# Kimahriman/hdfs-native

Hardware: AMD Instinct MI355X
Metric: GiB/s device-resident RS(6,3) encode+decode, 1 MiB cells, at 1/2/4/8 MI355X (higher is better)
Workload: dtype u8

## Files before the change

hdfs-native_amd/csrc/ec_kernels.hip:

```cpp
#include <hip/hip_runtime.h>

#include <dlfcn.h>

#include <algorithm>
#include <cstdint>
#include <functional>
#include <map>
#include <memory>
#include <mutex>
#include <thread>
#include <tuple>
#include <vector>

#include "bitslice.hpp"
#include "ec_kernels.hpp"
#include "gf_device.hpp"
#include "work_queue.hpp"
#include "xor_networks.hpp"

namespace hec {

template <int K, int R, int U, bool NT, int BS, int WQ = 0>
__global__ __launch_bounds__(BS) void gf_matmul_v16(MatmulArgs a) {
    static_assert(WQ == 0 || K > 0, "the work queue needs compile-time k");
    __shared__ PermTable s_tab[R][kMaxK];
    __shared__ uint8_t s_exp[512];
    __shared__ uint8_t s_log[256];
    __shared__ uint8_t s_coef[R * kMaxK];
    const int k = K ? K : a.k;
    prologue<R, BS>(a, k, s_tab, s_exp, s_log, s_coef);

    const uint32_t chunks = a.chunks;
    const uint32_t total = a.total_tiles;
    constexpr uint32_t TILE = WQ ? 64 * U : BS * U;
    constexpr uint32_t USTEP = WQ ? 64 : BS;
    const uint32_t lcol = WQ ? (threadIdx.x & 63u) : threadIdx.x;

    u32x4 acc[U][R];
#pragma unroll
    for (int u = 0; u < U; u++)
#pragma unroll
        for (int j = 0; j < R; j++) acc[u][j] = u32x4{0, 0, 0, 0};
    const uint32_t wq_n = gridDim.x < kMixedQueues ? gridDim.x : kMixedQueues;
    const uint32_t wq_q = blockIdx.x % wq_n;
    uint32_t* const wq_ctr = WQ ? a.queue + wq_q * (kMixedQueueStride / 4) : nullptr;
    if constexpr (WQ > 0) queue_zero_next(a.queue_zero);
    uint32_t wq_next, wq_round = 0, wq_left = 0;
    asm volatile("" : "=v"(wq_next));
    auto next_tile = [&]() -> uint32_t {
        for (;;) {
            if (wq_left == 0) {
                const uint32_t v = uint32_t(__builtin_amdgcn_readfirstlane(int(wq_next)));
                wq_round = v * uint32_t(WQ);
                wq_left = WQ;
                if (uint64_t(wq_round) * wq_n + wq_q >= total) return total;
                if ((threadIdx.x & 63u) == 0) wq_next = atomicAdd(wq_ctr, 1u);
            } else {
                wq_round++;
            }
            wq_left--;
            const uint64_t t = uint64_t(wq_round) * wq_n + wq_q;
            if (t < total) return uint32_t(t);
            wq_left = 0;
        }
    };
    if constexpr (WQ > 0)
        if ((threadIdx.x & 63u) == 0) wq_next = atomicAdd(wq_ctr, 1u);
    for (uint32_t tile = WQ ? next_tile() : blockIdx.x; tile < total; tile = WQ ? next_tile() : tile + gridDim.x) {
        uint32_t stripe, tcol;
        tile_coords(tile, a, stripe, tcol);
        asm volatile("" ::: "memory");
        if constexpr (K > 0) {
            u32x4 x[U][K];
            bool live[U];
            uint32_t offs[U];
#pragma unroll
            for (int u = 0; u < U; u++) {
                const uint32_t col = tcol * TILE + u * USTEP + lcol;
                live[u] = col < chunks;
                offs[u] = (live[u] ? col : 0u) * 16u;
            }
#pragma unroll
            for (int u = 0; u < U; u++)
#pragma unroll
                for (int i = 0; i < K; i++)
                    x[u][i] = load16<NT>((a.in[i] + uint64_t(stripe) * a.in_stride[i]) + offs[u]);
#pragma unroll
            for (int u = 0; u < U; u++)
#pragma unroll
                for (int j = 0; j < R; j++) asm volatile("" ::"v"(acc[u][j]));
            __builtin_amdgcn_sched_barrier(0);
#pragma unroll
            for (int i = 0; i < K; i++) {
                uint32_t toff = uint32_t(i) * uint32_t(sizeof(PermTable));
                asm volatile("" : "+v"(toff));
                if (i > 0) {
#pragma unroll
                    for (int u = 0; u < U; u++)
#pragma unroll
                        for (int j = 0; j < R; j++) asm volatile("" : "+v"(acc[u][j]) : "v"(toff));
                }
                Sel s[U][4];
#pragma unroll
                for (int u = 0; u < U; u++)
#pragma unroll
                    for (int d = 0; d < 4; d++) s[u][d] = make_sel(x[u][i][d]);
#pragma unroll
                for (int j = 0; j < R; j++) {
                    const PermTable& t =
                        *reinterpret_cast<const PermTable*>(reinterpret_cast<const char*>(&s_tab[j][0]) + toff);
                    const uint32_t t0lo = t.t0lo, t0hi = t.t0hi, t1lo = t.t1lo, t1hi = t.t1hi, t2 = t.t2;
#pragma unroll
                    for (int u = 0; u < U; u++)
#pragma unroll
                        for (int d = 0; d < 4; d++) {
                            const uint32_t p = gf_mul4(t0lo, t0hi, t1lo, t1hi, t2, s[u][d].s0, s[u][d].s1, s[u][d].s2);
                            acc[u][j][d] = i == 0 ? p : (acc[u][j][d] ^ p);
                        }
                }
                __builtin_amdgcn_sched_barrier(0);
            }
#pragma unroll
            for (int u = 0; u < U; u++)
#pragma unroll
                for (int j = 0; j < R; j++) asm volatile("" : "+v"(acc[u][j]));
            if ((tcol + 1) * TILE <= chunks) {
#pragma unroll
                for (int u = 0; u < U; u++)
#pragma unroll
                    for (int j = 0; j < R; j++)
                        store16<NT>((a.out[j] + uint64_t(stripe) * a.out_stride[j]) + offs[u], acc[u][j]);
            } else {
#pragma unroll
                for (int u = 0; u < U; u++) {
                    if (!live[u]) continue;
#pragma unroll
                    for (int j = 0; j < R; j++)
                        store16<NT>((a.out[j] + uint64_t(stripe) * a.out_stride[j]) + offs[u], acc[u][j]);
                }
            }
            if (a.drain) asm volatile("s_waitcnt vmcnt(0)" ::: "memory");
        } else {
#pragma unroll
            for (int u = 0; u < U; u++) {
                const uint32_t col = tcol * TILE + u * BS + threadIdx.x;
                if (col >= chunks) continue;
                const uint64_t off = uint64_t(col) * 16u;
                u32x4 racc[R];
#pragma unroll
                for (int j = 0; j < R; j++) racc[j] = u32x4{0, 0, 0, 0};
                for (int i = 0; i < k; i++) {
                    u32x4 x = load16<NT>(a.in[i] + uint64_t(stripe) * a.in_stride[i] + off);
                    Sel s[4];
#pragma unroll
                    for (int d = 0; d < 4; d++) s[d] = make_sel(x[d]);
#pragma unroll
                    for (int j = 0; j < R; j++) {
                        const PermTable& t = s_tab[j][i];
                        const uint32_t t0lo = t.t0lo, t0hi = t.t0hi, t1lo = t.t1lo, t1hi = t.t1hi, t2 = t.t2;
#pragma unroll
                        for (int d = 0; d < 4; d++)
                            racc[j][d] ^= gf_mul4(t0lo, t0hi, t1lo, t1hi, t2, s[d].s0, s[d].s1, s[d].s2);
                    }
                }
#pragma unroll
                for (int j = 0; j < R; j++) store16<NT>(a.out[j] + uint64_t(stripe) * a.out_stride[j] + off, racc[j]);
            }
        }
    }
}

template <int K, int R, int U, int BS>
__global__ __launch_bounds__(BS) void gf_encode_bsl(MatmulArgs a) {
    static_assert(bitslice::rs_net_available<K, R>() && U % 2 == 0, "bit-sliced RS encode");
    constexpr int G = U / 2;
    const uint32_t chunks = a.chunks;
    const uint32_t total = a.total_tiles;
    constexpr uint32_t TILE = BS * U;
    u32x4 acc[U][R];
#pragma unroll
    for (int u = 0; u < U; u++)
#pragma unroll
        for (int j = 0; j < R; j++) acc[u][j] = u32x4{0, 0, 0, 0};
    for (uint32_t tile = blockIdx.x; tile < total; tile += gridDim.x) {
        uint32_t stripe, tcol;
        tile_coords(tile, a, stripe, tcol);
        u32x4 x[U][K];
        bool live[U];
        uint32_t offs[U];
#pragma unroll
        for (int u = 0; u < U; u++) {
            const uint32_t col = tcol * TILE + u * BS + threadIdx.x;
            live[u] = col < chunks;
            offs[u] = (live[u] ? col : 0u) * 16u;
        }
#pragma unroll
        for (int u = 0; u < U; u++)
#pragma unroll
            for (int i = 0; i < K; i++) x[u][i] = load16<true>((a.in[i] + uint64_t(stripe) * a.in_stride[i]) + offs[u]);
#pragma unroll
        for (int u = 0; u < U; u++)
#pragma unroll
            for (int j = 0; j < R; j++) asm volatile("" ::"v"(acc[u][j]));
        __builtin_amdgcn_sched_barrier(0);
        uint32_t accp[G][R * 8];
#pragma unroll
        for (int i = 0; i < K; i++) {
#pragma unroll
            for (int g = 0; g < G; g++) {
                uint32_t pl[8] = {x[2 * g][i][0],     x[2 * g][i][1],     x[2 * g][i][2],     x[2 * g][i][3],
                                  x[2 * g + 1][i][0], x[2 * g + 1][i][1], x[2 * g + 1][i][2], x[2 * g + 1][i][3]};
                if (i > 0) {
#pragma unroll
                    for (int t = 0; t < R * 8; t++) asm volatile("" : "+v"(accp[g][t]));
                }
                bitslice::transpose8(pl);
                bitslice::rs_absorb_at<K, R>(i, pl, accp[g]);
                __builtin_amdgcn_sched_barrier(0);
            }
        }
#pragma unroll
        for (int g = 0; g < G; g++)
#pragma unroll
            for (int j = 0; j < R; j++) {
                uint32_t q[8];
#pragma unroll
                for (int t = 0; t < 8; t++) q[t] = accp[g][8 * j + t];
                bitslice::transpose8(q);
                acc[2 * g][j] = u32x4{q[0], q[1], q[2], q[3]};
                acc[2 * g + 1][j] = u32x4{q[4], q[5], q[6], q[7]};
            }
#pragma unroll
        for (int u = 0; u < U; u++)
#pragma unroll
            for (int j = 0; j < R; j++) asm volatile("" : "+v"(acc[u][j]));
        if ((tcol + 1) * TILE <= chunks) {
#pragma unroll
            for (int u = 0; u < U; u++)
#pragma unroll
                for (int j = 0; j < R; j++)
                    store16<true>((a.out[j] + uint64_t(stripe) * a.out_stride[j]) + offs[u], acc[u][j]);
        } else {
#pragma unroll
            for (int u = 0; u < U; u++) {
                if (!live[u]) continue;
#pragma unroll
                for (int j = 0; j < R; j++)
                    store16<true>((a.out[j] + uint64_t(stripe) * a.out_stride[j]) + offs[u], acc[u][j]);
            }
        }
        if (a.drain) asm volatile("s_waitcnt vmcnt(0)" ::: "memory");
    }
}

template <int K, int R, int U, int BS, bool BSL = false>
__global__ __launch_bounds__(BS) void gf_matmul_dma(MatmulArgs a) {
    static_assert(K > 0, "DMA kernel needs a compile-time input count");
    static_assert(!BSL || (bitslice::rs_net_available<K, R>() && U % 2 == 0), "bit-sliced RS encode");
    constexpr int WAVES = BS / 64;
    constexpr int PIECE = 1024;
    constexpr int STAGE = WAVES * K * U * PIECE;
    constexpr int TAB = R * kMaxK * int(sizeof(PermTable));
    __shared__ __attribute__((aligned(16))) uint8_t s_mem[STAGE + TAB + 512 + 256 + R * kMaxK];
    PermTable(*s_tab)[kMaxK] = reinterpret_cast<PermTable(*)[kMaxK]>(s_mem + STAGE);
    uint8_t* s_exp = s_mem + STAGE + TAB;
    uint8_t* s_log = s_exp + 512;
    uint8_t* s_coef = s_log + 256;
    prologue<R, BS>(a, K, s_tab, s_exp, s_log, s_coef);

    const uint32_t chunks = a.chunks;
    const uint32_t total = a.total_tiles;
    constexpr uint32_t TILE = BS * U;
    const int wave = __builtin_amdgcn_readfirstlane(threadIdx.x / 64);
    const int lane = threadIdx.x & 63;
    uint8_t* stage = s_mem + wave * (K * U * PIECE);

    auto issue = [&](uint32_t tile) {
        uint32_t stripe, tcol;
        tile_coords(tile, a, stripe, tcol);
#pragma unroll
        for (int u = 0; u < U; u++) {
            uint32_t col = tcol * TILE + u * BS + wave * 64 + lane;
            col = col < chunks ? col : chunks - 1;
            const uint32_t off = col * 16u;
#pragma unroll
            for (int i = 0; i < K; i++) {
                const uint8_t* src = (a.in[i] + uint64_t(stripe) * a.in_stride[i]) + off;
                __builtin_amdgcn_global_load_lds(
                    reinterpret_cast<const void*>(src),
                    (__attribute__((address_space(3))) void*)(stage + (i * U + u) * PIECE), 16, 0,
                    2 );
            }
        }
    };

    uint32_t tile = blockIdx.x;
    if (tile < total) issue(tile);
    bool prev_full = false;
    for (; tile < total; tile += gridDim.x) {
        if (prev_full)
            asm volatile("s_waitcnt vmcnt(%0)" ::"n"(R * U) : "memory");
        else
            asm volatile("s_waitcnt vmcnt(0)" ::: "memory");
        u32x4 x[U][K];
#pragma unroll
        for (int u = 0; u < U; u++)
#pragma unroll
            for (int i = 0; i < K; i++)
                x[u][i] = *reinterpret_cast<const u32x4*>(stage + (i * U + u) * PIECE + lane * 16);
        asm volatile("s_waitcnt lgkmcnt(0)" ::: "memory");
        __builtin_amdgcn_sched_barrier(0);
        const uint32_t next = tile + gridDim.x;
        if (next < total) issue(next);
        __builtin_amdgcn_sched_barrier(0);

        uint32_t stripe, tcol;
        tile_coords(tile, a, stripe, tcol);
        u32x4 acc[U][R];
        if constexpr (BSL) {
            constexpr int G = U / 2;
            uint32_t accp[G][R * 8];
#pragma unroll
            for (int i = 0; i < K; i++) {
#pragma unroll
                for (int g = 0; g < G; g++) {
                    uint32_t pl[8] = {x[2 * g][i][0],     x[2 * g][i][1],     x[2 * g][i][2],     x[2 * g][i][3],
                                      x[2 * g + 1][i][0], x[2 * g + 1][i][1], x[2 * g + 1][i][2], x[2 * g + 1][i][3]};
                    if (i > 0) {
#pragma unroll
                        for (int t = 0; t < R * 8; t++) asm volatile("" : "+v"(accp[g][t]));
                    }
                    bitslice::transpose8(pl);
                    bitslice::rs_absorb_at<K, R>(i, pl, accp[g]);
                    __builtin_amdgcn_sched_barrier(0);
                }
            }
#pragma unroll
            for (int g = 0; g < G; g++)
#pragma unroll
                for (int j = 0; j < R; j++) {
                    uint32_t q[8];
#pragma unroll
                    for (int t = 0; t < 8; t++) q[t] = accp[g][8 * j + t];
                    bitslice::transpose8(q);
                    acc[2 * g][j] = u32x4{q[0], q[1], q[2], q[3]};
                    acc[2 * g + 1][j] = u32x4{q[4], q[5], q[6], q[7]};
                }
        } else {
#pragma unroll
        for (int u = 0; u < U; u++)
#pragma unroll
            for (int j = 0; j < R; j++) acc[u][j] = u32x4{0, 0, 0, 0};
#pragma unroll
        for (int i = 0; i < K; i++) {
            uint32_t toff = uint32_t(i) * uint32_t(sizeof(PermTable));
            asm volatile("" : "+v"(toff));
#pragma unroll
            for (int u = 0; u < U; u++)
#pragma unroll
                for (int j = 0; j < R; j++) asm volatile("" : "+v"(acc[u][j]) : "v"(toff));
            Sel sl[U][4];
#pragma unroll
            for (int u = 0; u < U; u++)
#pragma unroll
                for (int d = 0; d < 4; d++) sl[u][d] = make_sel(x[u][i][d]);
#pragma unroll
            for (int j = 0; j < R; j++) {
                const PermTable& t =
                    *reinterpret_cast<const PermTable*>(reinterpret_cast<const char*>(&s_tab[j][0]) + toff);
                const uint32_t t0lo = t.t0lo, t0hi = t.t0hi, t1lo = t.t1lo, t1hi = t.t1hi, t2 = t.t2;
#pragma unroll
                for (int u = 0; u < U; u++)
#pragma unroll
                    for (int d = 0; d < 4; d++)
                        acc[u][j][d] ^= gf_mul4(t0lo, t0hi, t1lo, t1hi, t2, sl[u][d].s0, sl[u][d].s1, sl[u][d].s2);
            }
            __builtin_amdgcn_sched_barrier(0);
        }
        }
        const bool full = __builtin_amdgcn_readfirstlane(
                              int(tcol * TILE + (U - 1) * BS + wave * 64 + 63 < chunks)) != 0;
        if (full) {
#pragma unroll
            for (int u = 0; u < U; u++) {
                const uint32_t off = (tcol * TILE + u * BS + threadIdx.x) * 16u;
#pragma unroll
                for (int j = 0; j < R; j++)
                    store16<true>((a.out[j] + uint64_t(stripe) * a.out_stride[j]) + off, acc[u][j]);
            }
        } else {
#pragma unroll
            for (int u = 0; u < U; u++) {
                const uint32_t col = tcol * TILE + u * BS + threadIdx.x;
                if (col >= chunks) continue;
                const uint32_t off = col * 16u;
#pragma unroll
                for (int j = 0; j < R; j++)
                    store16<true>((a.out[j] + uint64_t(stripe) * a.out_stride[j]) + off, acc[u][j]);
            }
        }
        prev_full = full;
    }
    asm volatile("s_waitcnt vmcnt(0)" ::: "memory");
}

template <int K, int R, int U, int BS, bool RESIDENT, bool MIXED_SKIP = true, int WQ = 0>
__global__ __launch_bounds__(BS) void gf_decode_mixed(MixedArgs a) {
    static_assert(WQ == 0 || RESIDENT, "the work queue needs resident plans");
    static_assert(K > 0, "compile-time k");
    __shared__ PermTable s_tab[RESIDENT ? 1 : R][K];
    __shared__ DevPlanHeader s_hdr;
    __shared__ uint64_t s_base[kMaxShards], s_stride[kMaxShards], s_obase[kMaxK], s_ostride[kMaxK];
    extern __shared__ __attribute__((aligned(16))) uint8_t s_dyn[];
    const int tid = threadIdx.x;
    if (tid < kMaxShards) {
        s_base[tid] = reinterpret_cast<uint64_t>(a.base[tid]);
        s_stride[tid] = a.stride[tid];
    }
    if (tid < kMaxK) {
        s_obase[tid] = reinterpret_cast<uint64_t>(a.out[tid]);
        s_ostride[tid] = a.out_stride[tid];
    }
    const uint32_t off_bytes = (uint32_t(a.stripes) * 4u + 15u) & ~15u;
    if constexpr (RESIDENT) {
        const uint32_t off_words = uint32_t(a.stripes);
        for (uint32_t t = tid; t < off_words; t += BS) reinterpret_cast<uint32_t*>(s_dyn)[t] = a.stripe_off[t];
        const uint32_t words = a.blob_bytes / 4;
        for (uint32_t t = tid; t < words; t += BS)
            reinterpret_cast<uint32_t*>(s_dyn + off_bytes)[t] = reinterpret_cast<const uint32_t*>(a.plans)[t];
    }
    __syncthreads();
    const uint32_t chunks = a.chunks;
    const uint32_t total = a.total_tiles;
    constexpr uint32_t TILE = WQ ? 64 * U : BS * U;
    constexpr uint32_t USTEP = WQ ? 64 : BS;
    const uint32_t lcol = WQ ? (threadIdx.x & 63u) : threadIdx.x;
    MatmulArgs order;
    order.tiles_per_stripe = a.tiles_per_stripe;
    order.group = a.group;
    order.grouped_tiles = a.grouped_tiles;
    order.stripes = a.stripes;

    uint32_t t_begin = blockIdx.x, t_end = total, t_step = gridDim.x;
    if constexpr (!RESIDENT) {
        const uint32_t per = (total + gridDim.x - 1) / gridDim.x;
        t_begin = blockIdx.x * per;
        t_end = min(total, t_begin + per);
        t_step = 1;
        order.group = 1;
    }
    uint32_t cur_stripe = 0xFFFFFFFFu;
    bool cur_none = true;
    u32x4 acc[U][R];
#pragma unroll
    for (int u = 0; u < U; u++)
#pragma unroll
        for (int j = 0; j < R; j++) acc[u][j] = u32x4{0, 0, 0, 0};
    auto run_tile = [&](uint32_t tile) {
        uint32_t stripe, tcol;
        tile_coords(tile, order, stripe, tcol);
        const DevPlanHeader* hdr = &s_hdr;
        const PermTable* tabs = &s_tab[0][0];
        if constexpr (RESIDENT) {
            const uint32_t off = __builtin_amdgcn_readfirstlane(reinterpret_cast<const uint32_t*>(s_dyn)[stripe]);
            if (off == kNoPlan) return;
            hdr = reinterpret_cast<const DevPlanHeader*>(s_dyn + off_bytes + off);
            tabs = reinterpret_cast<const PermTable*>(s_dyn + off_bytes + off + sizeof(DevPlanHeader)) + a.row0 * K;
        } else {
            if (stripe != cur_stripe) {
                __syncthreads();
// ... 547 lines not shown
Shape default_shape(int k, uint64_t cell_len) {
    if (k > 6) return {2, 512, 8, true, false};
    (void)k;
    (void)cell_len;
    return {4, 256, 1, true, false};
}

}

namespace {

constexpr size_t kSetBytes = size_t(kMixedQueues) * kMixedQueueStride;
constexpr size_t kMaxStreamSets = 4096;
constexpr size_t kGraphSets = 256;

struct StreamSets {
    std::mutex mu;
    uint32_t* set[2] = {nullptr, nullptr};
    unsigned cur = 0;
    bool zeroed = false;
};

struct DeviceQueues {
    std::mutex mu;
    std::map<unsigned long long, std::unique_ptr<StreamSets>> streams;
    std::vector<std::unique_ptr<StreamSets>> thread_sets;
    uint32_t* graph_pool = nullptr;
    size_t graph_next = 0;
    bool reserved = false;
};

DeviceQueues& device_queues(int device) {
    static std::mutex mu;
    static std::map<int, std::unique_ptr<DeviceQueues>> all;
    std::lock_guard<std::mutex> lk(mu);
    auto& d = all[device];
    if (!d) d.reset(new DeviceQueues);
    return *d;
}

}

QueueLease::QueueLease(QueueLease&& o) noexcept : use(o.use), zero(o.zero), st_(o.st_) {
    o.use = o.zero = nullptr;
    o.st_ = nullptr;
}

QueueLease& QueueLease::operator=(QueueLease&& o) noexcept {
    if (this != &o) {
        if (st_) static_cast<StreamSets*>(st_)->mu.unlock();
        use = o.use;
        zero = o.zero;
        st_ = o.st_;
        o.use = o.zero = nullptr;
        o.st_ = nullptr;
    }
    return *this;
}

QueueLease::~QueueLease() {
    if (st_) static_cast<StreamSets*>(st_)->mu.unlock();
}

void QueueLease::launched() {
    if (st_) static_cast<StreamSets*>(st_)->cur ^= 1u;
}

void queue_reserve(int device) {
    DeviceQueues& d = device_queues(device);
    std::lock_guard<std::mutex> lk(d.mu);
    if (d.reserved) return;
    d.reserved = true;
    void* p = nullptr;
    if (hipMalloc(&p, kGraphSets * kSetBytes) != hipSuccess) {
        (void)hipGetLastError();
        return;
    }
    d.graph_pool = static_cast<uint32_t*>(p);
}

void queue_stats(int device, uint64_t* streams, uint64_t* graph_sets) {
    DeviceQueues& d = device_queues(device);
    std::lock_guard<std::mutex> lk(d.mu);
    if (streams) *streams = d.streams.size() + d.thread_sets.size();
    if (graph_sets) *graph_sets = d.graph_next;
}

namespace {

typedef hipError_t (*StreamGetIdFn)(hipStream_t, unsigned long long*);

StreamGetIdFn stream_get_id() {
    static const StreamGetIdFn fn = []() -> StreamGetIdFn {
        Dl_info info;
        if (!dladdr(reinterpret_cast<void*>(&hipMemsetAsync), &info) || !info.dli_fname) return nullptr;
        void* h = dlopen(info.dli_fname, RTLD_LAZY | RTLD_NOLOAD);
        if (!h) return nullptr;
        void* f = dlsym(h, "hipStreamGetId");
        dlclose(h);
        return reinterpret_cast<StreamGetIdFn>(f);
    }();
    return fn;
}

std::unique_ptr<StreamSets> make_sets() {
    std::unique_ptr<StreamSets> n(new StreamSets);
    void* p = nullptr;
    if (hipMalloc(&p, 2 * kSetBytes) != hipSuccess) {
        (void)hipGetLastError();
        return nullptr;
    }
    n->set[0] = static_cast<uint32_t*>(p);
    n->set[1] = n->set[0] + kSetBytes / 4;
    return n;
}

}

int queue_keyed_by_id() { return stream_get_id() ? 1 : 0; }

__global__ __launch_bounds__(256) void zero_words(unsigned long long* p, uint64_t n) {
    for (uint64_t i = uint64_t(blockIdx.x) * 256u + threadIdx.x; i < n; i += uint64_t(gridDim.x) * 256u) p[i] = 0ull;
}

hipError_t zero_async(void* p, size_t bytes, hipStream_t stream) {
    if (bytes == 0) return hipSuccess;
    hipStreamCaptureStatus cap = hipStreamCaptureStatusNone;
    if (hipStreamIsCapturing(stream, &cap) != hipSuccess) (void)hipGetLastError();
    if (cap != hipStreamCaptureStatusActive || (reinterpret_cast<uintptr_t>(p) | bytes) % 8 != 0)
        return hipMemsetAsync(p, 0, bytes, stream);
    unsigned long long* words = static_cast<unsigned long long*>(p);
    uint64_t n = bytes / 8;
    uint64_t grid = (n + 255) / 256;
    if (grid > 1024) grid = 1024;
    void* args[] = {&words, &n};
    return hipLaunchKernel(reinterpret_cast<const void*>(&zero_words), dim3(uint32_t(grid)), dim3(256), args, 0,
                           stream);
}

QueueLease queue_lease(int device, hipStream_t stream) {
    QueueLease l;
    hipStreamCaptureStatus cap = hipStreamCaptureStatusNone;
    if (hipStreamIsCapturing(stream, &cap) != hipSuccess) {
        (void)hipGetLastError();
        return l;
    }
    DeviceQueues& d = device_queues(device);
    if (cap != hipStreamCaptureStatusNone) {
        if (cap != hipStreamCaptureStatusActive) return l;
        uint32_t* set = nullptr;
        {
            std::lock_guard<std::mutex> lk(d.mu);
            if (d.graph_pool && d.graph_next < kGraphSets) set = d.graph_pool + d.graph_next++ * (kSetBytes / 4);
        }
        if (!set) return l;
        if (zero_async(set, kSetBytes, stream) != hipSuccess) {
            (void)hipGetLastError();
            return l;
        }
        l.use = set;
        return l;
    }
    StreamSets* st = nullptr;
    if (stream == hipStreamPerThread) {
        thread_local std::map<int, StreamSets*> mine;
        StreamSets*& t = mine[device];
        if (!t) {
            std::lock_guard<std::mutex> lk(d.mu);
            if (d.streams.size() + d.thread_sets.size() >= kMaxStreamSets) return l;
            std::unique_ptr<StreamSets> n = make_sets();
            if (!n) return l;
            t = n.get();
            d.thread_sets.push_back(std::move(n));
        }
        st = t;
    } else {
        unsigned long long key = reinterpret_cast<uintptr_t>(stream);
        if (StreamGetIdFn get_id = stream_get_id()) {
            if (get_id(stream, &key) != hipSuccess) {
                (void)hipGetLastError();
                return l;
            }
        }
        std::lock_guard<std::mutex> lk(d.mu);
        auto it = d.streams.find(key);
        if (it != d.streams.end()) {
            st = it->second.get();
        } else if (d.streams.size() + d.thread_sets.size() < kMaxStreamSets) {
            std::unique_ptr<StreamSets> n = make_sets();
            if (!n) return l;
            st = n.get();
            d.streams.emplace(key, std::move(n));
        }
    }
    if (!st) return l;
    st->mu.lock();
    if (!st->zeroed) {
        if (hipMemsetAsync(st->set[0], 0, 2 * kSetBytes, stream) != hipSuccess) {
            (void)hipGetLastError();
            st->mu.unlock();
            return l;
        }
        st->zeroed = true;
    }
    l.st_ = st;
    l.use = st->set[st->cur];
    l.zero = st->set[st->cur ^ 1u];
    return l;
}

bool rs_parity_matrix(const MatmulArgs& a) {
    if (a.k < 1 || a.k > kMaxK || a.r < 1 || a.r > kMaxR) return false;
    for (int j = 0; j < a.r; j++)
        for (int i = 0; i < a.k; i++) {
            const uint8_t s = uint8_t(a.k + j) ^ uint8_t(i);
            if (a.coef[j * kMaxK + i] != (s == 0 ? 0 : gf_div(1, s))) return false;
        }
    return true;
}

int launch_gf_matmul(const MatmulArgs& in, int device, hipStream_t stream) {
    MatmulArgs a = in;
    const Tune tn = tune_snapshot();
    bool aligned = true;
    for (int i = 0; i < a.k; i++)
        aligned &= ((reinterpret_cast<uintptr_t>(a.in[i]) | a.in_stride[i]) & 15u) == 0;
    for (int j = 0; j < a.r; j++)
        aligned &= ((reinterpret_cast<uintptr_t>(a.out[j]) | a.out_stride[j]) & 15u) == 0;
    const uint64_t chunks = (aligned && a.cell_len < (uint64_t(1) << 32)) ? a.cell_len / 16 : 0;
    const int cus = num_cus(device);

    if (chunks > 0) {
        Shape sh = default_shape(a.k, a.cell_len);
        if (tn.unroll) sh.unroll = tn.unroll == 3 ? 2 : tn.unroll;
        if (tn.block) sh.block = tn.block;
        if (tn.nt >= 0) sh.nt = tn.nt != 0;
        if (tn.blocks_per_cu) sh.blocks_per_cu = tn.blocks_per_cu;
        if (tn.pipeline == 1 || tn.pipeline == 2) sh.dma = tn.pipeline == 2;
        if (sh.block == 512 && sh.unroll > 2) sh.unroll = 2;
        const bool dma_ok = (a.k == 2 || a.k == 3 || a.k == 6 || a.k == 10);
        if (sh.dma && !dma_ok) sh.dma = false;
        if (sh.dma) {
            if (a.k == 10) {
                sh.unroll = 2;
                sh.block = 256;
            } else if (sh.block == 512) {
                sh.unroll = 2;
            } else if (sh.unroll < 2) {
                sh.unroll = 2;
            }
        }
        const void* fn = nullptr;
        QueueLease lease;
        const int tile_mult = 1;
#ifdef HEC_EXPERIMENTAL
        if (!fn && tn.matmul_bsl == 1 && sh.unroll % 2 == 0 && rs_parity_matrix(a))
            fn = sh.dma ? pick_dma_bsl(a.k, a.r, sh.unroll, sh.block) : pick_bsl(a.k, a.r, sh);
#endif
        int wq = 0;
        bool pair = false;
        if (!fn && tn.matmul_pair == 1 && sh.nt) {
            const void* f = pick_pair(a.k, a.r);
            if (f) lease = queue_lease(device, stream);
            if (f && lease) {
                fn = f;
                pair = true;
                wq = 1;
                a.queue = lease.use;
                a.queue_zero = lease.zero;
                sh.unroll = 4;
                sh.block = 128;
                if (!tn.blocks_per_cu) sh.blocks_per_cu = 4;
            }
        }
        const bool k10_256 = kExperimental && a.k == 10 && sh.block == 256 && (sh.unroll == 2 || sh.unroll == 4);
        if (!fn && !pair && !sh.dma && sh.nt &&
            ((sh.unroll == (sh.block == 512 ? 2 : 4) && (sh.block == 512) == (a.k == 10)) || k10_256)) {
            wq = default_wq(a.k);
            if (kExperimental && tn.matmul_wq) wq = tn.matmul_wq == 3 ? 0 : tn.matmul_wq;
            const void* f = wq ? pick_wq(a.k, a.r, wq, sh.block, sh.unroll) : nullptr;
            if (f) lease = queue_lease(device, stream);
            a.queue = lease.use;
            a.queue_zero = lease.zero;
            if (a.queue) {
                fn = f;
                if (!tn.blocks_per_cu) sh.blocks_per_cu = 1;
            } else {
                wq = 0;
            }
        }
        if (!fn) fn = sh.dma ? pick_dma(a.k, a.r, sh.unroll, sh.block) : pick_vec(a.k, a.r, sh);
        if (!fn) return -1;
        const uint64_t tile = uint64_t(wq ? 64 : sh.block) * sh.unroll * tile_mult;
        const uint64_t tps = (chunks + tile - 1) / tile;
        const uint64_t total = tps * a.stripes;
        if (chunks > 0xFFFFFFFFull || total > 0xFFF00000ull) return -1;
        a.chunks = uint32_t(chunks);
        a.tiles_per_stripe = uint32_t(tps);
        a.total_tiles = uint32_t(total);
        tile_order(a.stripes, a.tiles_per_stripe, tn.group > 0 ? uint32_t(tn.group) : 4u, a.group, a.grouped_tiles);
        a.drain = tn.drain == 1 ? 0u : 1u;
        uint64_t grid = tn.grid ? uint64_t(tn.grid) : uint64_t(cus) * sh.blocks_per_cu;
        if (grid > total) grid = total;
        void* args[] = {&a};
        const hipError_t e = hipLaunchKernel(fn, dim3(uint32_t(grid)), dim3(sh.block), args, 0, stream);
        if (e != hipSuccess) return int(e);
        lease.launched();
    }
    uint64_t begin = chunks * 16;
    if (begin == 0 && !aligned && a.cell_len >= 8 && a.r >= 1 && a.r <= kMaxR && tn.unaligned != 1) {
        const uint64_t total = (a.cell_len / 8) * a.stripes;
        uint64_t grid = (total + 255) / 256;
        const uint64_t cap = uint64_t(cus) * 8;
        if (grid > cap) grid = cap;
        const void* fn = a.r == 1   ? reinterpret_cast<const void*>(&gf_matmul_dw<1>)
                         : a.r == 2 ? reinterpret_cast<const void*>(&gf_matmul_dw<2>)
                         : a.r == 3 ? reinterpret_cast<const void*>(&gf_matmul_dw<3>)
                                    : reinterpret_cast<const void*>(&gf_matmul_dw<4>);
        void* args[] = {&a};
        const hipError_t e = hipLaunchKernel(fn, dim3(uint32_t(grid)), dim3(256), args, 0, stream);
        if (e != hipSuccess) return int(e);
        begin = (a.cell_len / 8) * 8;
    }
    if (begin < a.cell_len) {
        a.byte_begin = begin;
        const uint64_t total = (a.cell_len - begin) * a.stripes;
        uint64_t grid = (total + kBlock - 1) / kBlock;
        const uint64_t cap = uint64_t(cus) * 8;
        if (grid > cap) grid = cap;
        void* args[] = {&a};
        const hipError_t e = hipLaunchKernel(reinterpret_cast<const void*>(&gf_matmul_bytes), dim3(uint32_t(grid)),
                                             dim3(kBlock), args, 0, stream);
        if (e != hipSuccess) return int(e);
    }
    const hipError_t e = hipGetLastError();
    return e == hipSuccess ? 0 : int(e);
}

namespace {

template <int K, int R, bool RES, bool SKIP, int WQ = 0>
const void* mixed_fn() {
    if constexpr (K > 6)
        return reinterpret_cast<const void*>(&gf_decode_mixed<K, R, 2, 512, RES, SKIP, WQ>);
    else
        return reinterpret_cast<const void*>(&gf_decode_mixed<K, R, 4, 256, RES, SKIP, WQ>);
}

template <int K, int R>
const void* mixed_sel(bool res, bool skip, int wq) {
    if (res && skip && wq == 1) return mixed_fn<K, R, true, true, 1>();
    if (res && skip && wq == 4) return mixed_fn<K, R, true, true, 4>();
#ifdef HEC_EXPERIMENTAL
    if (res && skip && wq == 2) return mixed_fn<K, R, true, true, 2>();
    return res ? (skip ? mixed_fn<K, R, true, true>() : mixed_fn<K, R, true, false>())
               : (skip ? mixed_fn<K, R, false, true>() : mixed_fn<K, R, false, false>());
#else
    (void)skip;
    return res ? mixed_fn<K, R, true, true>() : mixed_fn<K, R, false, true>();
#endif
}

template <int K>
const void* mixed_pick_r(int r, bool res, bool skip, int wq) {
    switch (r) {
        case 1: return mixed_sel<K, 1>(res, skip, wq);
        case 2: return mixed_sel<K, 2>(res, skip, wq);
        case 3: return mixed_sel<K, 3>(res, skip, wq);
        default: return mixed_sel<K, 4>(res, skip, wq);
    }
}

constexpr uint64_t kResidentMax = 156u << 10;
constexpr uint64_t kDynNoAttr = 64u << 10;

}

int launch_decode_mixed(const MixedArgs& in, int rows, int device, hipStream_t stream) {
    MixedArgs a = in;
    const Tune tn = tune_snapshot();
    if (a.cell_len % 16 != 0 || a.cell_len / 16 > 0xFFFFFFFFull) return -1;
    const uint64_t dyn = ((a.stripes * 4 + 15) & ~uint64_t(15)) + a.blob_bytes;
    bool res = dyn <= kResidentMax && a.blob_bytes % 4 == 0;
    const bool skip = tn.mixed_skip != 1;
    int wq = (a.queue && skip) ? (a.k >= 6 ? 1 : 4) : 0;
    if (kExperimental && tn.mixed_wq) wq = tn.mixed_wq == 3 ? 0 : tn.mixed_wq;
    auto pick = [&](bool resident) -> const void* {
        const int w = resident ? wq : 0;
        switch (a.k) {
            case 2: return mixed_pick_r<2>(rows, resident, skip, w);
            case 3: return mixed_pick_r<3>(rows, resident, skip, w);
            case 6: return mixed_pick_r<6>(rows, resident, skip, w);
            case 10: return mixed_pick_r<10>(rows, resident, skip, w);
            default: return nullptr;
        }
    };
    const void* fn = pick(res);
    if (!fn) return -1;
    if (res && dyn > kDynNoAttr &&
        hipFuncSetAttribute(fn, hipFuncAttributeMaxDynamicSharedMemorySize, int(kResidentMax)) != hipSuccess) {
        (void)hipGetLastError();
        res = false;
        fn = pick(false);
    }
    if (!res) wq = 0;
    const int U = a.k > 6 ? 2 : 4, BS = a.k > 6 ? 512 : 256;
    const int bpc = tn.blocks_per_cu ? tn.blocks_per_cu : (a.k > 6 ? 8 : 1);
    const uint64_t chunks = a.cell_len / 16;
    const uint64_t tile = uint64_t(wq ? 64 : BS) * U;
    const uint64_t tps = (chunks + tile - 1) / tile;
    const uint64_t total = tps * a.stripes;
    if (total > 0xFFFFFFFFull) return -1;
    if (total == 0) return 0;
    a.chunks = uint32_t(chunks);
    a.tiles_per_stripe = uint32_t(tps);
    a.total_tiles = uint32_t(total);
    tile_order(a.stripes, a.tiles_per_stripe, tn.group > 0 ? uint32_t(tn.group) : 4u, a.group, a.grouped_tiles);
    a.drain = tn.drain == 1 ? 0u : 1u;
    uint64_t grid = uint64_t(num_cus(device)) * (wq && !tn.blocks_per_cu ? 1 : bpc);
    if (grid > total) grid = total;
    void* args[] = {&a};
    const hipError_t e = hipLaunchKernel(fn, dim3(uint32_t(grid)), dim3(BS), args, res ? uint32_t(dyn) : 0u, stream);
    return e == hipSuccess ? 0 : int(e);
}

}
```

hdfs-native_amd/csrc/ec_kernels.hpp:

```cpp
#pragma once

#ifndef __HIPCC_RTC__
#include <hip/hip_runtime.h>
#else
typedef struct ihipStream_t* hipStream_t;
#endif

#include <cstdint>

#include "tuning.hpp"

namespace hec {

constexpr int kBlock = 256;
constexpr int kMaxK = 32;
constexpr int kMaxR = 4;

struct MatmulArgs {
    const uint8_t* in[kMaxK];
    uint64_t in_stride[kMaxK];
    uint8_t* out[kMaxR];
    uint64_t out_stride[kMaxR];
    uint8_t coef[kMaxR * kMaxK];
    int32_t k;
    int32_t r;
    uint64_t cell_len;
    uint64_t stripes;
    uint64_t byte_begin;
    uint32_t chunks;
    uint32_t tiles_per_stripe;
    uint32_t total_tiles;
    uint32_t group;
    uint32_t grouped_tiles;
    uint32_t drain;
    uint32_t col_rot = 0;
    uint32_t* queue = nullptr;
    uint32_t* queue_zero = nullptr;
};

struct PermTable {
    uint32_t t0lo, t0hi, t1lo, t1hi, t2, pad0, pad1, pad2;
};

constexpr int kMaxShards = kMaxK + 16;

struct DevPlanHeader {
    uint32_t e;
    uint8_t surv[kMaxK];
    uint8_t miss[16];
    uint8_t pad[12];
};
static_assert(sizeof(DevPlanHeader) == 64, "plan header is 64 B");

constexpr uint32_t kNoPlan = 0xFFFFFFFFu;

constexpr uint32_t kMixedQueues = 8, kMixedQueueStride = 256;
constexpr size_t kMixedQueueBytes = size_t(16) * kMixedQueues * kMixedQueueStride;
struct MixedArgs {
    const uint8_t* base[kMaxShards];
    uint64_t stride[kMaxShards];
    uint8_t* out[kMaxK];
    uint64_t out_stride[kMaxK];
    const uint8_t* plans;
    const uint32_t* stripe_off;
    uint32_t blob_bytes;
    int32_t k;
    int32_t row0;
    uint64_t cell_len;
    uint64_t stripes;
    uint32_t chunks, tiles_per_stripe, total_tiles, group, grouped_tiles;
    uint32_t drain;
    uint32_t* queue;
};

#ifndef __HIPCC_RTC__
struct QueueLease {
    uint32_t* use = nullptr;
    uint32_t* zero = nullptr;
    QueueLease() = default;
    QueueLease(QueueLease&& o) noexcept;
    QueueLease& operator=(QueueLease&& o) noexcept;
    QueueLease(const QueueLease&) = delete;
    QueueLease& operator=(const QueueLease&) = delete;
    ~QueueLease();
    explicit operator bool() const { return use != nullptr; }
    void launched();
    void* st_ = nullptr;
};
QueueLease queue_lease(int device, hipStream_t stream);
void queue_reserve(int device);
hipError_t zero_async(void* p, size_t bytes, hipStream_t stream);
void queue_stats(int device, uint64_t* streams, uint64_t* graph_sets);
int queue_keyed_by_id();
#endif

int launch_decode_mixed(const MixedArgs& a, int rows, int device, hipStream_t stream);

struct ReconArgs {
    const uint8_t* base[kMaxShards];
    uint64_t stride[kMaxShards];
    uint8_t* out[kMaxShards];
    uint64_t out_stride[kMaxShards];
    const uint8_t* plans;
    const uint32_t* stripe_off;
    uint32_t blob_bytes;
    int32_t k;
    int32_t row0;
    uint64_t cell_len;
    uint64_t stripes;
    uint32_t chunks, tiles_per_stripe, total_tiles, group, grouped_tiles;
    uint32_t drain;
    uint32_t* queue;
};

int launch_reconstruct_mixed(const ReconArgs& a, int rows, int device, hipStream_t stream);
constexpr uint64_t kReconResidentMax = 156u << 10;
inline bool mixed_resident(uint64_t stripes, uint64_t blob_bytes) {
    return ((stripes * 4 + 15) & ~uint64_t(15)) + blob_bytes <= kReconResidentMax && blob_bytes % 4 == 0;
}

struct ScrubArgs {
    const uint8_t* base[kMaxShards];
    uint64_t stride[kMaxShards];
    uint8_t coef[16 * kMaxK];
    int32_t k, m;
    uint64_t cell_len;
    uint64_t stripes;
    uint64_t* results;
    uint32_t chunks, tiles_per_stripe, total_tiles, group, grouped_tiles;
    uint32_t drain;
    uint32_t* queue;
    uint32_t* queue_zero;
};

int launch_scrub(const ScrubArgs& a, int device, hipStream_t stream);

struct ScrubPlanHeader {
    uint32_t e;
    uint8_t surv[kMaxK];
    uint8_t extras[16];
    uint32_t missing_lo;
    uint32_t missing_hi;
    uint8_t pad[4];
};
static_assert(sizeof(ScrubPlanHeader) == 64, "plan header is 64 B");

struct ScrubMixedArgs {
    const uint8_t* base[kMaxShards];
    uint64_t stride[kMaxShards];
    const uint8_t* plans;
    const uint32_t* stripe_off;
    uint32_t blob_bytes;
    int32_t k;
    uint64_t cell_len;
    uint64_t stripes;
    uint64_t* results;
    uint32_t chunks, tiles_per_stripe, total_tiles, group, grouped_tiles;
    uint32_t drain;
    uint32_t* queue;
};

int launch_scrub_mixed(const ScrubMixedArgs& a, int max_e, int device, hipStream_t stream);
int launch_scrub_mixed_bytes(const ScrubMixedArgs& a, int device, hipStream_t stream);

bool rs_parity_matrix(const MatmulArgs& a);

int launch_gf_matmul(const MatmulArgs& a, int device, hipStream_t stream);


}
```

hdfs-native_amd/csrc/gf_device.hpp:

```cpp
#pragma once

#ifndef __HIPCC_RTC__
#include <hip/hip_runtime.h>
#endif

#include <cstdint>

#include "ec_kernels.hpp"
#include "gf256.hpp"
#include "work_queue.hpp"

namespace hec {
namespace {

typedef uint32_t u32x4 __attribute__((ext_vector_type(4)));

__constant__ GfTables kDevGf = GfTables();


__device__ __forceinline__ uint8_t lds_gf_mul(const uint8_t* s_exp, const uint8_t* s_log, uint8_t a,
                                              uint8_t b) {
    return (a == 0 || b == 0) ? 0 : s_exp[s_log[a] + s_log[b]];
}

__device__ __forceinline__ uint32_t pack4(uint8_t a, uint8_t b, uint8_t c, uint8_t d) {
    return uint32_t(a) | (uint32_t(b) << 8) | (uint32_t(c) << 16) | (uint32_t(d) << 24);
}

__device__ void build_perm_table(PermTable* t, uint8_t c, const uint8_t* s_exp, const uint8_t* s_log) {
    uint8_t p0[8], p1[8], p2[4];
#pragma unroll
    for (int e = 0; e < 8; e++) {
        p0[e] = lds_gf_mul(s_exp, s_log, c, uint8_t(e));
        p1[e] = lds_gf_mul(s_exp, s_log, c, uint8_t(e << 3));
    }
#pragma unroll
    for (int e = 0; e < 4; e++) p2[e] = lds_gf_mul(s_exp, s_log, c, uint8_t(e << 6));
    t->t0lo = pack4(p0[0], p0[1], p0[2], p0[3]);
    t->t0hi = pack4(p0[4], p0[5], p0[6], p0[7]);
    t->t1lo = pack4(p1[0], p1[1], p1[2], p1[3]);
    t->t1hi = pack4(p1[4], p1[5], p1[6], p1[7]);
    t->t2 = pack4(p2[0], p2[1], p2[2], p2[3]);
    t->pad0 = t->pad1 = t->pad2 = 0;
}

__device__ __forceinline__ uint32_t xor3(uint32_t a, uint32_t b, uint32_t c) {
    return __builtin_amdgcn_bitop3_b32(a, b, c, 0x96);
}

__device__ __forceinline__ uint32_t gf_mul4(uint32_t t0lo, uint32_t t0hi, uint32_t t1lo, uint32_t t1hi,
                                            uint32_t t2, uint32_t s0, uint32_t s1, uint32_t s2) {
    uint32_t a = __builtin_amdgcn_perm(t0hi, t0lo, s0);
    uint32_t b = __builtin_amdgcn_perm(t1hi, t1lo, s1);
    uint32_t c = __builtin_amdgcn_perm(t2, t2, s2);
    return xor3(a, b, c);
}

struct Sel {
    uint32_t s0, s1, s2;
};

__device__ __forceinline__ void tile_coords(uint32_t tile, const MatmulArgs& a, uint32_t& stripe, uint32_t& tcol) {
    const uint32_t tps = a.tiles_per_stripe;
    const uint32_t G = a.group;
    if (G <= 1 || tile >= a.grouped_tiles) {
        stripe = tile / tps;
        tcol = tile - stripe * tps;
        return;
    }
    const uint32_t per_group = G * tps;
    const uint32_t g = tile / per_group;
    const uint32_t r = tile - g * per_group;
    tcol = r / G;
    stripe = g * G + (r - tcol * G);
}

__host__ inline void tile_order(uint64_t stripes, uint32_t tiles_per_stripe, uint32_t want, uint32_t& group,
                                uint32_t& grouped_tiles) {
    group = uint32_t(want < 1 ? 1 : (stripes < want ? (stripes < 1 ? 1 : stripes) : want));
    grouped_tiles = uint32_t((stripes / group) * group * tiles_per_stripe);
}

__device__ __forceinline__ Sel make_sel(uint32_t x) {
    Sel s;
    s.s0 = x & 0x07070707u;
    s.s1 = (x >> 3) & 0x07070707u;
    s.s2 = (x >> 6) & 0x03030303u;
    return s;
}

template <bool NT>
__device__ __forceinline__ u32x4 load16(const uint8_t* p) {
    if constexpr (NT)
        return __builtin_nontemporal_load(reinterpret_cast<const u32x4*>(p));
    else
        return *reinterpret_cast<const u32x4*>(p);
}

template <bool NT>
__device__ __forceinline__ void store16(uint8_t* p, u32x4 v) {
    if constexpr (NT)
        __builtin_nontemporal_store(v, reinterpret_cast<u32x4*>(p));
    else
        *reinterpret_cast<u32x4*>(p) = v;
}

__device__ __forceinline__ uint64_t uniform64(uint64_t v) {
    const uint32_t lo = uint32_t(__builtin_amdgcn_readfirstlane(int(uint32_t(v))));
    const uint32_t hi = uint32_t(__builtin_amdgcn_readfirstlane(int(uint32_t(v >> 32))));
    return uint64_t(lo) | (uint64_t(hi) << 32);
}

typedef __attribute__((address_space(1))) uint8_t gbyte;
typedef __attribute__((address_space(1))) u32x4 gu32x4;

__device__ __forceinline__ const gbyte* gptr(uint64_t a) { return reinterpret_cast<const gbyte*>(a); }
__device__ __forceinline__ gbyte* gptr_w(uint64_t a) { return reinterpret_cast<gbyte*>(a); }

__device__ __forceinline__ u32x4 gload16(const gbyte* p) {
    return __builtin_nontemporal_load(reinterpret_cast<const gu32x4*>(p));
}
__device__ __forceinline__ void gstore16(gbyte* p, u32x4 v) {
    __builtin_nontemporal_store(v, reinterpret_cast<gu32x4*>(p));
}

template <int R, int BS, int KC = kMaxK>
__device__ __forceinline__ void prologue(const MatmulArgs& a, int k, PermTable (*s_tab)[KC], uint8_t* s_exp,
                                         uint8_t* s_log, uint8_t* s_coef) {
    static_assert(BS >= 256 && BS % 256 == 0, "prologue assumes >= 256 threads");
    const int tid = threadIdx.x;
    if (tid < 256) {
        s_exp[tid] = kDevGf.exp[tid];
        s_exp[tid + 256] = kDevGf.exp[tid + 256];
        s_log[tid] = kDevGf.log[tid];
    }
    if (tid < R * kMaxK) s_coef[tid] = a.coef[tid];
    __syncthreads();
    for (int t = tid; t < R * k; t += BS) {
        int j = t / k, i = t - j * k;
        build_perm_table(&s_tab[j][i], s_coef[j * kMaxK + i], s_exp, s_log);
    }
    __syncthreads();
}

}
}
```

hdfs-native_amd/csrc/work_queue.hpp:

```cpp
#pragma once

#ifndef __HIPCC_RTC__
#include <hip/hip_runtime.h>
#endif

#include <cstdint>

#include "ec_kernels.hpp"

namespace hec {
namespace {

__device__ __forceinline__ void queue_zero_next(uint32_t* zero) {
    if (zero && blockIdx.x == 0 && threadIdx.x < kMixedQueues) zero[threadIdx.x * (kMixedQueueStride / 4)] = 0u;
}

struct WaveQueue {
    uint32_t* ctr;
    uint32_t n, q, total, pend, peek_v;
    bool peeked;
    __device__ __forceinline__ void init(uint32_t* queue, uint32_t total_tiles) {
        n = gridDim.x < kMixedQueues ? gridDim.x : kMixedQueues;
        q = blockIdx.x % n;
        total = total_tiles;
        ctr = queue + q * (kMixedQueueStride / 4);
        peeked = false;
        asm volatile("" : "=v"(pend));
        if ((threadIdx.x & 63u) == 0) pend = atomicAdd(ctr, 1u);
    }
    __device__ __forceinline__ uint32_t tile_of(uint32_t v) const {
        const uint64_t t = uint64_t(v) * n + q;
        return t < total ? uint32_t(t) : total;
    }
    __device__ __forceinline__ uint32_t peek() {
        if (!peeked) {
            peek_v = uint32_t(__builtin_amdgcn_readfirstlane(int(pend)));
            peeked = true;
        }
        return tile_of(peek_v);
    }
    __device__ __forceinline__ uint32_t next() {
        const uint32_t v = peeked ? peek_v : uint32_t(__builtin_amdgcn_readfirstlane(int(pend)));
        peeked = false;
        const uint32_t t = tile_of(v);
        if (t < total && (threadIdx.x & 63u) == 0) pend = atomicAdd(ctr, 1u);
        return t;
    }
};

}
}
```

Before: 3904.

## Precompute GF tables on host and overlap first tile loads with prologue

For the work-queue matmul kernel, the permutation tables are now built on the host and passed in the kernel argument block, so each block copies words into shared memory instead of rebuilding tables from exp/log lookups. With the K=10 static-first mode, each wave takes its first tile statically (the queue base is offset accordingly) and issues that tile's loads before storing the tables and syncing, which hides the prologue under memory latency. Load issue and compute are split into lambdas so the next tile's loads are issued right after the current tile is computed. This enlarges the kernel argument block and makes the queue counter arithmetic more involved.

Result: no change. 3913 (median of 6 runs) (+0.2%).

```diff
diff --git a/hdfs-native_amd/csrc/ec_kernels.hip b/hdfs-native_amd/csrc/ec_kernels.hip
--- a/hdfs-native_amd/csrc/ec_kernels.hip
+++ b/hdfs-native_amd/csrc/ec_kernels.hip
@@ -20,15 +20,35 @@
 
 namespace hec {
 
+#ifndef HEC_WQ_STATIC_FIRST
+#define HEC_WQ_STATIC_FIRST 1
+#endif
+template <int WQ>
+struct MatmulKernelArgs {
+    typedef MatmulWqArgs type;
+    static __device__ __forceinline__ const MatmulArgs& plain(const MatmulWqArgs& w) { return w.a; }
+};
+template <>
+struct MatmulKernelArgs<0> {
+    typedef MatmulArgs type;
+    static __device__ __forceinline__ const MatmulArgs& plain(const MatmulArgs& a) { return a; }
+};
+
 template <int K, int R, int U, bool NT, int BS, int WQ = 0>
-__global__ __launch_bounds__(BS) void gf_matmul_v16(MatmulArgs a) {
+__global__ __launch_bounds__(BS) void gf_matmul_v16(typename MatmulKernelArgs<WQ>::type args) {
     static_assert(WQ == 0 || K > 0, "the work queue needs compile-time k");
+    constexpr bool STATIC_FIRST = WQ > 0 && (HEC_WQ_STATIC_FIRST == 2 || (HEC_WQ_STATIC_FIRST == 1 && K == 10));
+    const MatmulArgs& a = MatmulKernelArgs<WQ>::plain(args);
     __shared__ PermTable s_tab[R][kMaxK];
-    __shared__ uint8_t s_exp[512];
-    __shared__ uint8_t s_log[256];
-    __shared__ uint8_t s_coef[R * kMaxK];
     const int k = K ? K : a.k;
-    prologue<R, BS>(a, k, s_tab, s_exp, s_log, s_coef);
+    if constexpr (WQ == 0) {
+        __shared__ uint8_t s_exp[512];
+        __shared__ uint8_t s_log[256];
+        __shared__ uint8_t s_coef[R * kMaxK];
+        prologue<R, BS>(a, k, s_tab, s_exp, s_log, s_coef);
+    } else if constexpr (!STATIC_FIRST) {
+        prologue_tables<K, R>(args, s_tab);
+    }
 
     const uint32_t chunks = a.chunks;
     const uint32_t total = a.total_tiles;
@@ -44,13 +64,14 @@
     const uint32_t wq_n = gridDim.x < kMixedQueues ? gridDim.x : kMixedQueues;
     const uint32_t wq_q = blockIdx.x % wq_n;
     uint32_t* const wq_ctr = WQ ? a.queue + wq_q * (kMixedQueueStride / 4) : nullptr;
-    if constexpr (WQ > 0) queue_zero_next(a.queue_zero);
+    const uint32_t wq_base = STATIC_FIRST ? uint32_t(BS / 64) * queue_blocks(gridDim.x, wq_n, wq_q) : 0u;
+    if constexpr (WQ > 0 && !STATIC_FIRST) queue_zero_next(a.queue_zero);
     uint32_t wq_next, wq_round = 0, wq_left = 0;
     asm volatile("" : "=v"(wq_next));
     auto next_tile = [&]() -> uint32_t {
         for (;;) {
             if (wq_left == 0) {
-                const uint32_t v = uint32_t(__builtin_amdgcn_readfirstlane(int(wq_next)));
+                const uint32_t v = uint32_t(__builtin_amdgcn_readfirstlane(int(wq_next))) + wq_base;
                 wq_round = v * uint32_t(WQ);
                 wq_left = WQ;
                 if (uint64_t(wq_round) * wq_n + wq_q >= total) return total;
@@ -64,16 +85,14 @@
             wq_left = 0;
         }
     };
-    if constexpr (WQ > 0)
-        if ((threadIdx.x & 63u) == 0) wq_next = atomicAdd(wq_ctr, 1u);
-    for (uint32_t tile = WQ ? next_tile() : blockIdx.x; tile < total; tile = WQ ? next_tile() : tile + gridDim.x) {
-        uint32_t stripe, tcol;
+    uint32_t stripe = 0, tcol = 0;
+    u32x4 x[U][K ? K : 1];
+    bool live[U];
+    uint32_t offs[U];
+    auto issue = [&](uint32_t tile) __attribute__((always_inline)) {
         tile_coords(tile, a, stripe, tcol);
         asm volatile("" ::: "memory");
         if constexpr (K > 0) {
-            u32x4 x[U][K];
-            bool live[U];
-            uint32_t offs[U];
 #pragma unroll
             for (int u = 0; u < U; u++) {
                 const uint32_t col = tcol * TILE + u * USTEP + lcol;
@@ -90,6 +109,10 @@
 #pragma unroll
                 for (int j = 0; j < R; j++) asm volatile("" ::"v"(acc[u][j]));
             __builtin_amdgcn_sched_barrier(0);
+        }
+    };
+    auto code = [&]() __attribute__((always_inline)) {
+        if constexpr (K > 0) {
 #pragma unroll
             for (int i = 0; i < K; i++) {
                 uint32_t toff = uint32_t(i) * uint32_t(sizeof(PermTable));
@@ -166,6 +189,36 @@
 #pragma unroll
                 for (int j = 0; j < R; j++) store16<NT>(a.out[j] + uint64_t(stripe) * a.out_stride[j] + off, racc[j]);
             }
+        }
+    };
+    if constexpr (!STATIC_FIRST) {
+        if constexpr (WQ > 0)
+            if ((threadIdx.x & 63u) == 0) wq_next = atomicAdd(wq_ctr, 1u);
+        for (uint32_t tile = WQ ? next_tile() : blockIdx.x; tile < total;
+             tile = WQ ? next_tile() : tile + gridDim.x) {
+            issue(tile);
+            code();
+        }
+    } else {
+        const uint32_t wave = uint32_t(__builtin_amdgcn_readfirstlane(int(threadIdx.x >> 6)));
+        wq_round = ((blockIdx.x / wq_n) * uint32_t(BS / 64) + wave) * uint32_t(WQ);
+        wq_left = WQ - 1;
+        const uint64_t t0 = uint64_t(wq_round) * wq_n + wq_q;
+        uint32_t tile = t0 < total ? uint32_t(t0) : total;
+        const uint32_t word = prologue_table_load<K, R>(args);
+        if (tile < total) {
+            issue(tile);
+            if ((threadIdx.x & 63u) == 0) wq_next = atomicAdd(wq_ctr, 1u);
+            queue_zero_next(a.queue_zero);
+            prologue_table_store<K, R>(word, s_tab);
+            while (tile < total) {
+                code();
+                tile = next_tile();
+                if (tile < total) issue(tile);
+            }
+        } else {
+            queue_zero_next(a.queue_zero);
+            prologue_table_store<K, R>(word, s_tab);
         }
     }
 }
@@ -1319,7 +1372,13 @@
         a.drain = tn.drain == 1 ? 0u : 1u;
         uint64_t grid = tn.grid ? uint64_t(tn.grid) : uint64_t(cus) * sh.blocks_per_cu;
         if (grid > total) grid = total;
-        void* args[] = {&a};
+        MatmulWqArgs w;
+        const bool wq_tables = wq && !pair;
+        if (wq_tables) {
+            w.a = a;
+            fill_wq_tables(w);
+        }
+        void* args[] = {wq_tables ? static_cast<void*>(&w) : static_cast<void*>(&a)};
         const hipError_t e = hipLaunchKernel(fn, dim3(uint32_t(grid)), dim3(sh.block), args, 0, stream);
         if (e != hipSuccess) return int(e);
         lease.launched();
diff --git a/hdfs-native_amd/csrc/ec_kernels.hpp b/hdfs-native_amd/csrc/ec_kernels.hpp
--- a/hdfs-native_amd/csrc/ec_kernels.hpp
+++ b/hdfs-native_amd/csrc/ec_kernels.hpp
@@ -8,6 +8,7 @@
 
 #include <cstdint>
 
+#include "gf256.hpp"
 #include "tuning.hpp"
 
 namespace hec {
@@ -41,6 +42,27 @@
 struct PermTable {
     uint32_t t0lo, t0hi, t1lo, t1hi, t2, pad0, pad1, pad2;
 };
+
+constexpr int kWqMaxK = 10;
+constexpr int kWqTabWords = 5;
+struct MatmulWqArgs {
+    MatmulArgs a;
+    uint32_t tab[kMaxR][kWqMaxK][kWqTabWords];
+};
+static_assert(sizeof(MatmulWqArgs) == sizeof(MatmulArgs) + kMaxR * kWqMaxK * kWqTabWords * 4,
+              "the tables follow the plain block with no padding");
+static_assert(sizeof(MatmulWqArgs) <= 2048, "well under HIP's 4096-B kernel-argument limit");
+
+#ifndef __HIPCC_RTC__
+inline void fill_wq_tables(MatmulWqArgs& w) {
+    for (int j = 0; j < kMaxR; j++)
+        for (int i = 0; i < kWqMaxK; i++) {
+            const bool used = j < w.a.r && i < w.a.k;
+            const std::array<uint32_t, 8> t = perm_table_words(used ? w.a.coef[j * kMaxK + i] : 0);
+            for (int x = 0; x < kWqTabWords; x++) w.tab[j][i][x] = used ? t[x] : 0u;
+        }
+}
+#endif
 
 constexpr int kMaxShards = kMaxK + 16;
 
diff --git a/hdfs-native_amd/csrc/gf_device.hpp b/hdfs-native_amd/csrc/gf_device.hpp
--- a/hdfs-native_amd/csrc/gf_device.hpp
+++ b/hdfs-native_amd/csrc/gf_device.hpp
@@ -143,5 +143,36 @@
     __syncthreads();
 }
 
+template <int K, int R>
+__device__ __forceinline__ uint32_t prologue_table_load(const MatmulWqArgs& w) {
+    static_assert(K >= 1 && K <= kWqMaxK && R >= 1 && R <= kMaxR, "tables in the argument block");
+    static_assert(R * K * kWqTabWords <= 256, "one word per thread of the smallest block");
+    const uint32_t t = threadIdx.x;
+    uint32_t word = 0;
+    if (t < uint32_t(R * K * kWqTabWords)) {
+        const uint32_t j = t / uint32_t(K * kWqTabWords), r = t - j * uint32_t(K * kWqTabWords);
+        const uint32_t i = r / uint32_t(kWqTabWords), x = r - i * uint32_t(kWqTabWords);
+        word = w.tab[j][i][x];
+    }
+    return word;
+}
+
+template <int K, int R, int KC = kMaxK>
+__device__ __forceinline__ void prologue_table_store(uint32_t word, PermTable (*s_tab)[KC]) {
+    static_assert(K <= KC, "columns of s_tab");
+    const uint32_t t = threadIdx.x;
+    if (t < uint32_t(R * K * kWqTabWords)) {
+        const uint32_t j = t / uint32_t(K * kWqTabWords), r = t - j * uint32_t(K * kWqTabWords);
+        const uint32_t i = r / uint32_t(kWqTabWords), x = r - i * uint32_t(kWqTabWords);
+        reinterpret_cast<uint32_t*>(&s_tab[j][i])[x] = word;
+    }
+    __syncthreads();
+}
+
+template <int K, int R, int KC = kMaxK>
+__device__ __forceinline__ void prologue_tables(const MatmulWqArgs& w, PermTable (*s_tab)[KC]) {
+    prologue_table_store<K, R>(prologue_table_load<K, R>(w), s_tab);
+}
+
 }
 }
diff --git a/hdfs-native_amd/csrc/work_queue.hpp b/hdfs-native_amd/csrc/work_queue.hpp
--- a/hdfs-native_amd/csrc/work_queue.hpp
+++ b/hdfs-native_amd/csrc/work_queue.hpp
@@ -13,6 +13,10 @@
 
 __device__ __forceinline__ void queue_zero_next(uint32_t* zero) {
     if (zero && blockIdx.x == 0 && threadIdx.x < kMixedQueues) zero[threadIdx.x * (kMixedQueueStride / 4)] = 0u;
+}
+
+__device__ __forceinline__ uint32_t queue_blocks(uint32_t grid, uint32_t n, uint32_t q) {
+    return (grid - 1u - q) / n + 1u;
 }
 
 struct WaveQueue {
```
